# ChrisDud0257/SSL

Measured on AMD Instinct MI355X. Metric: SSG-loss edge-pixels/sec (fwd+bwd) 3x256x256 k_s=25 k_w=9, higher is better.
Workload: dtype f32; 1 GPU; C2: batch 16 x 3x256x256 per GPU, Laplacian mask, k_s=25 k_w=9 sigma=1.0, L1+KL w=1e3, SSGs materialised; launch=per-kernel, ranks_seen=1, edge_px_rank0=76466, images_rank0=16, input_checksum=c1391ff6908574f6, gradient_accumulation=fixed-point integer atomics (bit-reproducible, the shipped default), prewarm_steps=1949, parallelism=images sharded x1, no data-path collective

## Files before the change

include/ssg_hip.h:

```cpp
#ifndef SSG_HIP_H
#define SSG_HIP_H

#include <stddef.h>
#include <stdint.h>

#ifdef __cplusplus
extern "C" {
#endif

typedef void *ssg_stream_t;

#define SSG_E_BADARG (-1)
#define SSG_E_TOOLARGE (-2)
#define SSG_E_WORKSPACE (-3)
#define SSG_E_IMAGESMALL (-4)
#define SSG_E_ALIGN (-5)
#define SSG_E_PLAN (-6)

int ssg_abi_version(void);
const char *ssg_status_string(int status);
int ssg_device_status(ssg_stream_t stream);

int ssg_set_operator_plan_threshold(int positions);
int ssg_operator_pool_trim(void);
int ssg_compute_similarity(const float *image, const int *pos, float *out,
                           int mc, int psize, int ksize, int height, int width,
                           int channel, ssg_stream_t stream);

int ssg_compute_similarity_backward(const float *image, const float *grads,
                                    const int *pos, float *image_grads, int mc,
                                    int psize, int ksize, int height, int width,
                                    int channel, ssg_stream_t stream);

size_t ssg_edge_scratch_bytes(int B, int H, int W);
size_t ssg_forward_plan_bytes(int B, int H, int W, int capacity);
int ssg_set_dense_threshold(int edge_pixels_per_tile);
int ssg_set_overlap(int mode);
int ssg_last_overlap_assignment(void);
int ssg_set_tiny_step(int on);
int ssg_edge_list(const void *mask, int mask_kind, int mask_channels, int B,
                  int H, int W, int mask_stride, float lap_threshold,
                  int plan_ks ,
                  int *edges, int capacity, int *counts,
                  int *rank_map , int *tile_order ,
                  int *fwd_plan , void *scratch,
                  ssg_stream_t stream);

int ssg_edge_mask_laplacian(const float *gt, int B, int H, int W,
                            float lap_threshold, int mask_stride,
                            uint8_t *mask_out, ssg_stream_t stream);

int ssg_map_forward(const float *img, const float *img2, int B, int C, int H,
                    int W, const int *edges, const int *tile_order ,
                    const int *rank_map ,
// ... 113 lines not shown
```

ssl_amd/_lib.py:

```python
import ctypes
import os
import subprocess

_HERE = os.path.dirname(os.path.abspath(__file__))
CSRC = os.path.join(_HERE, "csrc")
SO_PATH = os.path.join(CSRC, "libssg_hip.so")
PROF_SO_PATH = os.path.join(CSRC, "libssg_hip_prof.so")
HEADER = os.path.join(os.path.dirname(_HERE), "include", "ssg_hip.h")

_vp, _i, _f, _sz = ctypes.c_void_p, ctypes.c_int, ctypes.c_float, ctypes.c_size_t

PROTOTYPES = {
    "ssg_abi_version": (_i, []),
    "ssg_status_string": (ctypes.c_char_p, [_i]),
    "ssg_compute_similarity": (_i, [_vp, _vp, _vp, _i, _i, _i, _i, _i, _i, _vp]),
    "ssg_compute_similarity_backward": (_i, [_vp, _vp, _vp, _vp, _i, _i, _i, _i, _i, _i, _vp]),
    "ssg_edge_scratch_bytes": (_sz, [_i, _i, _i]),
    "ssg_forward_plan_bytes": (_sz, [_i, _i, _i, _i]),
    "ssg_set_dense_threshold": (_i, [_i]),
    "ssg_set_overlap": (_i, [_i]),
    "ssg_last_overlap_assignment": (_i, []),
    "ssg_set_tiny_step": (_i, [_i]),
    "ssg_edge_list": (_i, [_vp, _i, _i, _i, _i, _i, _i, _f, _i, _vp, _i, _vp, _vp, _vp, _vp, _vp, _vp]),
    "ssg_edge_mask_laplacian": (_i, [_vp, _i, _i, _i, _f, _i, _vp, _vp]),
    "ssg_map_forward": (_i, [_vp, _vp, _i, _i, _i, _i, _vp, _vp, _vp, _vp, _vp, _i, _i, _i, _f, _f, _i, _vp, _vp,
                             _vp, _vp]),
    "ssg_backward_scratch_bytes": (_sz, [_i, _i]),
    "ssg_map_backward": (_i, [_vp, _i, _i, _i, _i, _vp, _vp, _vp, _vp, _vp, _i, _i, _i, _f, _i, _vp, _vp, _vp, _vp,
                              _vp, _vp]),
    "ssg_grad_fix_bytes": (_sz, [_i, _i, _i, _i]),
    "ssg_loss_scratch_bytes": (_sz, [_i, _i, _i, _i, _i]),
    "ssg_loss_backward": (_i, [_vp, _i, _i, _i, _i, _vp, _vp, _vp, _vp, _vp, _i, _i, _i, _f, _i, _vp, _vp, _f, _f,
                               _vp, _vp, _vp, _vp, _vp, _vp, _i, _vp]),
    "ssg_loss_workspace_bytes": (_sz, [_i, _i, _i, _i, _i]),
    "ssg_loss_rows_bytes": (_sz, [_i, _i]),
    "ssg_loss_tm_bytes": (_sz, [_i, _i]),
    "ssg_loss_workspace_layout": (_i, [_i, _i, _i, _i, _i, _i, ctypes.POINTER(ctypes.c_size_t)]),
# ... 102 lines not shown
```

ssl_amd/csrc/ssg_api.hip:

```cpp
#include "../../include/ssg_hip.h"

#include <atomic>
#include <cstdlib>
#include <mutex>

#include "ssg_common.hpp"

namespace ssg {
int launch_fwd(const FwdParams &p, hipStream_t st);
int launch_bwd(const BwdParams &p, hipStream_t st);
unsigned bwd_grid(const BwdParams &p);
size_t bwd_max_partials(int B, int H, int W, int n_rows);
int launch_loss_finalize(const LossFinalize &f, hipStream_t st);
const char *fwd_kernel_name(int ks, int kw);
const char *bwd_kernel_name(int ks, int kw);
size_t edge_scratch_bytes(int B, int H, int W);
int launch_edge_list(const void *mask, int kind, int mask_channels, int B, int H, int W, int stride, float thr,
                     int *edges, int capacity, int *counts, int *rank, int *order, int *plan, int dense_thr,
                     int plan_tile_rows, void *scratch, void *zero_a, size_t zero_a_bytes, void *zero_b,
                     size_t zero_b_bytes, void *zero_c, size_t zero_c_bytes, hipStream_t st);
size_t fwd_plan_bytes(int B, int H, int W, int capacity);
int fwd_plan_order_offset(int B, int H, int W);
struct DenseParams {
  const float *img[2];
  float *out[2];
  int nimg;
  const int *rank;
  const int *n_dense;
  const int *tiles;
  int max_tiles;
  const int *n_dev;
  int n_host;
  int B, H, W;
  float sigma, eps;
  int generalization;
  int dbg;
  double *row_scale;
  float *tm[2];
  int tm_slots;
  int grid_tiles;
  const int *strips;
  int max_strips;
  int *status;
  int raw;
};
int fwd_plan_strip_offset(int B, int H, int W);
int dense_max_strips(int B, int H, int W, int ks);
bool dense_supported(int ks, int kw, int C);
int dense_max_tiles(int B, int H, int W, int ks);
int dense_tile_rows(int ks);
int launch_fwd_dense(const DenseParams &p, int ks, int kw, int C, hipStream_t st);
int launch_edge_mask(const float *gt, int B, int H, int W, float thr, int stride, uint8_t *out, hipStream_t st);
bool grow_supported(int ks, int kw);
unsigned grow_grid(int n_host);
int launch_grad_rows(const GrowParams &p, int ks, int kw, hipStream_t st);
int launch_rows_tm(const TmRowsParams &p, int ks, int kw, hipStream_t st);
int rows_tm_parts(int n_tiles);
int launch_pos_to_mask(const int *pos, int mc, int Hp, int Wp, uint8_t *mask, hipStream_t st);
int launch_pos_relabel(const int *pos, int mc, int Hp, int Wp, int *rank, int *perm, int *dup, int *ndup, int *plan,
                       int *order2, hipStream_t st);
// ... 27 lines not shown

constexpr int DENSE_THR_DEFAULT = 16;
static std::atomic<int> g_dense_thr{-1};
static int dense_threshold() {
  int v = g_dense_thr.load(std::memory_order_relaxed);
  if (v < 0) {
    v = env_int("SSG_DENSE_THR", DENSE_THR_DEFAULT);
    if (v < 0) v = 0;
    g_dense_thr.store(v, std::memory_order_relaxed);
  }
  return v;
}

static std::atomic<int> g_tiny_step{1};
extern "C" int ssg_set_tiny_step(int on) { return g_tiny_step.exchange(on != 0 ? 1 : 0, std::memory_order_relaxed); }
extern "C" int ssg_set_operator_plan_threshold(int positions);
extern "C" int ssg_set_dense_threshold(int edge_pixels_per_tile) {
  const int prev = dense_threshold();
  g_dense_thr.store(edge_pixels_per_tile > 0 ? edge_pixels_per_tile : 0, std::memory_order_relaxed);
  return prev;
}

#ifdef SSG_PROFILE
static std::atomic<int> g_dbg{-1};
static int dbg_mask() {
  int v = g_dbg.load(std::memory_order_relaxed);
  if (v < 0) {
    v = env_int("SSG_DEBUG_SKIP", 0);
    if (v < 0) v = 0;
    g_dbg.store(v, std::memory_order_relaxed);
// ... 81 lines not shown
int *plan_hint_device_word(hipStream_t st) {
  if (overlap_mode() != 3) return nullptr;
  return plan_hint(stream_capturing(st)).dev;
}
}

struct Schedule {
  hipStream_t st = nullptr;
  bool may_fork = false;
  int assign = 0;
  bool chains = false;
  bool gated = false;
  int rows_hint = 0;
  SideStream *side = nullptr;
  bool open = false;
  hipStream_t dense() const { return open && assign == 2 ? side->side : st; }
  hipStream_t direct() const { return open && assign == 1 ? side->side : st; }
};

static Schedule schedule(hipStream_t st, int ks, bool chains) {
  Schedule s;
  s.st = st;
  const int mode = overlap_mode();
  int n_sparse = -1, n_tiles = -1;
  if (mode == 3) {
    const PlanHint h = plan_hint(true);
    if (h.host) {
      n_sparse = ((volatile int *)h.host)[0];
      n_tiles = ((volatile int *)h.host)[1];
    }
// ... 73 lines not shown

static int bwd_qsplit() {
  static int v = -1;
  if (v < 0) {
    v = env_int("SSG_BWD_QSPLIT", 0);
    if (v < 0) v = 0;
    if (v > 25) v = 25;
  }
  return v;
}

static size_t split_scratch_bytes(int n_rows, int ks) {
  const size_t n = (size_t)(n_rows > 0 ? n_rows : 1);
  return align_up(sizeof(float) * n * ks * ks, 256) + 3 * align_up(sizeof(float) * n, 256);
}

struct TileMajor {
  float *rows[2] = {nullptr, nullptr};
  int slots = 0;
};
static bool strips_enabled() {
  static int v = -1;
  if (v < 0) {
    v = env_int("SSG_STRIPS", 1) != 0;
  }
  return v != 0;
}
static bool tile_major_enabled() {
  static int v = -1;
  if (v < 0) {
// ... 3 lines not shown
}

static int split_tm_tiles(const BwdParams &p, const TileMajor *tm) {
  if (!tm || tm->slots <= 0) return 0;
  const int mt = dense_max_tiles(p.B, p.H, p.W, p.ks);
  return tm->slots < mt ? tm->slots : mt;
}

static bool split_row_classes(const BwdParams &p, int n_tm) {
  return p.mode == GRAD_LOSS && n_tm == 0 && p.row_scale && p.ks <= 25;
}

static int split_backward(BwdParams p, const int *rank, const int *plan, void *scratch, Schedule &sc,
                          const LossFinalize *fin = nullptr, bool *fin_done = nullptr, const TileMajor *tm = nullptr) {
  const hipStream_t st = sc.st;
  float *G = (float *)scratch;
  const size_t nfl = align_up(sizeof(float) * (size_t)(p.n_host > 0 ? p.n_host : 1), 256);
  float *sum_b = (float *)((char *)scratch + align_up(sizeof(float) * (size_t)p.n_host * p.ks * p.ks, 256));
  float *gmax_part = (float *)((char *)sum_b + nfl);
  float *dot = (float *)((char *)gmax_part + nfl);
  const int n_tm = split_tm_tiles(p, tm);
  GrowParams g{};
  g.mode = p.mode;
  g.gin = p.gin;
  g.ssg = p.ssg;
  g.ssg2 = p.ssg2;
  g.row_scale = p.row_scale;
  g.rows_scratch = p.rows_scratch;
  g.n_dev = p.n_dev;
  g.n_host = p.n_host;
  g.C = p.C;
  g.sigma = p.sigma;
  g.generalization = p.generalization;
  g.w_l1 = p.w_l1;
  g.w_kl = p.w_kl;
// ... 10 lines not shown
  }
  const size_t n_fix = (size_t)p.B * p.C * p.H * p.W;
  const bool apriori = p.gfix && p.mode == GRAD_LOSS && n_tm == 0;
  const bool classes = split_row_classes(p, n_tm);
  if (sc.chains && !sc.open && classes && p.grad) fork_side(sc, dbg_mask() & ((1 << 27) | (1 << 28) | (1 << 29)));
  const bool gated = sc.open && sc.gated;
  if (apriori) {
    g.gmax_part = nullptr;
    g.fix_word = (unsigned *)(p.gfix + n_fix);
  }
  int rc = gated ? (int)hipEventRecord(sc.side->gate, st) : 0;
  if (!rc && !(dbg_mask() & (1 << 29))) {
    if (classes) {
      GrowParams gd = g;
      gd.only = 1;
      rc = launch_grad_rows(gd, p.ks, p.kw, sc.dense());
      GrowParams gs = g;
      gs.only = 2;
      gs.grid_cap = 4096;
      gs.tm_hdr = plan + 1;
      gs.tm_slots = 0;
      gs.sparse_order = plan + fwd_plan_order_offset(p.B, p.H, p.W);
      gs.partials = p.partials + 2 * (size_t)grow_grid(p.n_host);
      if (!rc) rc = launch_grad_rows(gs, p.ks, p.kw, sc.direct());
    } else {
      rc = launch_grad_rows(g, p.ks, p.kw, st);
    }
  }
  if (!rc && n_tm > 0) {
    TmRowsParams t{};
    t.tm[0] = tm->rows[0];
// ... 354 lines not shown
}

int ssg_edge_list(const void *mask, int mask_kind, int mask_channels, int B, int H, int W, int mask_stride,
                  float lap_threshold, int plan_ks, int *edges, int capacity, int *counts, int *rank_map,
                  int *tile_order, int *fwd_plan, void *scratch, ssg_stream_t stream) {
  return edge_list_impl(mask, mask_kind, mask_channels, B, H, W, mask_stride, lap_threshold, plan_ks, edges, capacity,
                        counts, rank_map, tile_order, fwd_plan, scratch, nullptr, 0, nullptr, 0, nullptr, 0, stream);
}

int ssg_edge_mask_laplacian(const float *gt, int B, int H, int W, float lap_threshold, int mask_stride,
                            uint8_t *mask_out, ssg_stream_t stream) {
  if (!gt || !mask_out || B <= 0 || H <= 0 || W <= 0) return SSG_E_BADARG;
  return launch_edge_mask(gt, B, H, W, lap_threshold, mask_stride, mask_out, (hipStream_t)stream);
}

static int map_forward_impl(const float *img, const float *img2, int B, int C, int H, int W, const int *edges,
                            const int *tile_order, const int *rank_map, const int *fwd_plan, const int *n_edges_dev,
                            int n_rows, int ks, int kw, float sigma, float eps, int generalization, float *ssg,
                            float *ssg2, double *row_scale, bool row_scale_zeroed, Schedule &sc,
                            const TileMajor *tm = nullptr) {
  if (n_rows < 0 || !sizes_ok(ks, kw) || B <= 0 || C <= 0) return SSG_E_BADARG;
  if (H <= ks / 2 || W <= ks / 2) return SSG_E_IMAGESMALL;
  if (n_rows == 0) return 0;
  if (!img || !edges || !ssg || ((img2 != nullptr) != (ssg2 != nullptr))) return SSG_E_BADARG;
  FwdParams p{};
  p.img[0] = img;
  p.img[1] = img2;
  p.out[0] = ssg;
  p.out[1] = ssg2;
  p.nimg = img2 ? 2 : 1;
  p.edges = edges;
  p.estride = 3;
  p.order = tile_order;
  p.n_dev = n_edges_dev;
  p.n_host = n_rows;
// ... 18 lines not shown
    d.rank = rank_map;
    d.n_dense = fwd_plan + 1;
    d.tiles = fwd_plan + 4;
    d.max_tiles = dense_max_tiles(B, H, W, ks);
    d.n_dev = n_edges_dev;
    d.n_host = n_rows;
    d.B = B;
    d.H = H;
    d.W = W;
    d.sigma = sigma;
    d.eps = eps;
    d.generalization = generalization;
    d.dbg = (dbg_mask() >> 16) & 0xff;
    d.row_scale = row_scale;
    d.status = device_status_word();
    if (tm && tm->slots > 0 && row_scale && img2) {
      d.tm[0] = tm->rows[0];
      d.tm[1] = tm->rows[1];
      d.tm_slots = tm->slots;
      d.max_strips = strips_enabled() ? dense_max_strips(B, H, W, ks) : 0;
      d.strips = d.max_strips ? fwd_plan + fwd_plan_strip_offset(B, H, W) : nullptr;
    }
    if (row_scale && !row_scale_zeroed) {
      const int rc0 = (int)hipMemsetAsync(row_scale, 0, sizeof(double) * 2 * (size_t)n_rows, sc.st);
      if (rc0) return rc0;
    }
    fork_side(sc, dbg_mask() & ((1 << 25) | (1 << 26)));
    int rc = (dbg_mask() & (1 << 25)) ? 0 : launch_fwd_dense(d, ks, kw, C, sc.dense());
    p.order = fwd_plan + fwd_plan_order_offset(B, H, W);
    p.n_dev = fwd_plan;
// ... 51 lines not shown
    Schedule sc = schedule((hipStream_t)stream, ks, false);
    rc = split_backward(p, rank_map, fwd_plan, scratch, sc);
  } else {
    if (p.gfix) rc = launch_grad_fix_bound(p, (hipStream_t)stream);
    if (!rc) rc = launch_bwd(p, (hipStream_t)stream);
  }
  return rc ? rc : det_end(p, (hipStream_t)stream);
}

size_t ssg_grad_fix_bytes(int B, int C, int H, int W) { return sizeof(long long) * ((size_t)B * C * H * W + 8); }

static size_t partials_bytes(int B, int H, int W, int n_rows) {
  return align_up(2 * sizeof(float) * bwd_max_partials(B, H, W, n_rows) + 64, 256);
}

size_t ssg_loss_scratch_bytes(int B, int H, int W, int n_rows, int ks) {
  return partials_bytes(B, H, W, n_rows) + split_scratch_bytes(n_rows, ks);
}

static int loss_backward(const float *sr, int B, int C, int H, int W, const int *edges, const int *tile_order,
                         const int *rank_map, const int *fwd_plan, const int *n_edges_dev, int n_rows, int ks, int kw,
                         float sigma, int generalization, float *ssg_sr, float *ssg_gt, float w_l1, float w_kl,
                         const float *upstream, float *loss_out, float *grad_sr, void *scratch, void *grad_fix,
                         const double *row_scale, bool rows_scratch, bool fix_zeroed, bool grad_is_output,
                         Schedule &sc, const TileMajor *tm = nullptr, bool nan_on_overflow = false) {
  if (n_rows < 0 || !sizes_ok(ks, kw) || B <= 0 || C <= 0 || !loss_out) return SSG_E_BADARG;
  if (H <= ks / 2 || W <= ks / 2) return SSG_E_IMAGESMALL;
  const hipStream_t st = sc.st;
  if (n_rows == 0) return (int)hipMemsetAsync(loss_out, 0, 2 * sizeof(float), st);
  if (!sr || !edges || !ssg_sr || !ssg_gt || !scratch) return SSG_E_BADARG;
  BwdParams p{};
  p.img = sr;
// ... 17 lines not shown
  p.partials = (float *)scratch;
  p.upstream = upstream;
  p.ks = ks;
  p.kw = kw;
  p.dbg = (dbg_mask() >> 8) & 0xff;
  p.row_scale = row_scale;
  p.rows_scratch = rows_scratch ? 1 : 0;
  const bool split = split_ok(ks, kw, C, rank_map, fwd_plan, scratch);
  if (row_scale && !split) return SSG_E_BADARG;
  int rc = det_begin(p, grad_fix, st, fix_zeroed);
  if (rc) return rc;
  const int n_tm = split ? split_tm_tiles(p, tm) : 0;
  const int nparts = !split ? (int)bwd_grid(p)
                            : (split_row_classes(p, n_tm) ? 2 : 1) * (int)grow_grid(n_rows) + rows_tm_parts(n_tm);
  const int set_size = split && n_tm == 0 ? (int)grow_grid(n_rows) : 0;
  const LossFinalize fin{p.partials, nparts, n_edges_dev, n_rows, ks * ks, w_l1, w_kl, loss_out, nan_on_overflow ? 1 : 0, set_size};
  bool fin_done = false;
  if (split) {
    rc = split_backward(p, rank_map, fwd_plan, (char *)scratch + partials_bytes(B, H, W, n_rows), sc, &fin, &fin_done, tm);
  } else {
    p.fix_inline = p.gfix ? 1 : 0;
    rc = launch_bwd(p, st);
  }
  const int fin_reads = set_size > 0 ? (nparts / set_size) * ((n_rows + 3) / 4) : nparts;
  if (!rc) rc = det_end(p, st, grad_is_output, (fin_done || fin_reads > 8192) ? nullptr : &fin, &fin_done);
  if (rc || fin_done) return rc;
  return launch_loss_finalize(fin, st);
}

int ssg_loss_backward(const float *sr, int B, int C, int H, int W, const int *edges, const int *tile_order,
                      const int *rank_map, const int *fwd_plan, const int *n_edges_dev, int n_rows, int ks, int kw,
                      float sigma, int generalization,
                      float *ssg_sr, float *ssg_gt, float w_l1, float w_kl, const float *upstream,
                      float *loss_out, float *grad_sr, void *scratch, void *grad_fix, const double *row_scale,
                      int rows_are_scratch, ssg_stream_t stream) {
  Schedule sc = schedule((hipStream_t)stream, ks, true);
  const int rc = loss_backward(sr, B, C, H, W, edges, tile_order, rank_map, fwd_plan, n_edges_dev, n_rows, ks, kw, sigma,
                               generalization, ssg_sr, ssg_gt, w_l1, w_kl, upstream, loss_out, grad_sr, scratch,
                               grad_fix, row_scale, rows_are_scratch != 0, false, false, sc);
// ... 132 lines not shown
    t.dbg = env_int("SSG_TINY_DBG", 0);
    return launch_tiny_step(t, C, (hipStream_t)stream);
  }
  int *order = (int *)(ws + lw.order);
  int *plan = (int *)(ws + lw.plan);
  void *escratch = ws + lw.escratch;
  void *lscratch = ws + lw.lscratch;
  double *row_scale = (double *)(ws + lw.row_scale);
  const bool defer = split_ok(ks, kw, C, rank, plan, lscratch) && dense_supported(ks, kw, C);
  if (!defer) tm.slots = 0;
  if (defer) order = nullptr;
  if (!dense_supported(ks, kw, C)) plan = nullptr;
  const bool zero_fix = grad_fix && grad_sr;
  Schedule sc = schedule((hipStream_t)stream, ks, defer && grad_sr);
  const size_t fix_bytes = sizeof(long long) * ((size_t)B * C * H * W + 8), rs_bytes = 2 * sizeof(double) * (size_t)capacity;
  int rc = edge_list_impl(mask_kind == 2 ? (const void *)gt : mask, mask_kind, mask_kind == 2 ? 3 : mask_channels, B, H,
                          W, mask_stride, lap_threshold, ks, edges, capacity, counts, rank, order, plan, escratch,
                          defer ? (void *)row_scale : nullptr, rs_bytes, zero_fix ? grad_fix : nullptr, fix_bytes,
                          (grad_is_output && grad_sr && !zero_fix) ? (void *)grad_sr : nullptr,
                          sizeof(float) * (size_t)B * C * H * W, stream);
  if (!rc && grad_is_output && grad_sr && !zero_fix && ((sizeof(float) * (size_t)B * C * H * W) & 15))
    rc = (int)hipMemsetAsync((char *)grad_sr + ((sizeof(float) * (size_t)B * C * H * W) & ~(size_t)15), 0,
                             (sizeof(float) * (size_t)B * C * H * W) & 15, (hipStream_t)stream);
  if (rc) return rc;
  rc = map_forward_impl(sr, gt, B, C, H, W, edges, order, rank, plan, counts, capacity, ks, kw, sigma, eps,
                        generalization, ssg_sr, ssg_gt, defer ? row_scale : nullptr, defer, sc, &tm);
  if (!rc)
    rc = loss_backward(sr, B, C, H, W, edges, order, rank, plan, counts, capacity, ks, kw, sigma, generalization,
                       ssg_sr, ssg_gt, w_l1, w_kl, nullptr, loss_out, grad_sr, lscratch, grad_fix,
                       defer ? row_scale : nullptr, fused, zero_fix, grad_is_output && zero_fix, sc, &tm, true);
  const int rcj = join_side(sc);
  return rc ? rc : rcj;
}

int ssg_loss_fwd_bwd(const float *sr, const float *gt, const void *mask, int mask_kind, int mask_channels, int B,
                     int C, int H, int W, int ks, int kw, float sigma, float eps, int generalization, float w_l1,
                     float w_kl, int mask_stride, float lap_threshold, int capacity, float *ssg_sr, float *ssg_gt,
                     int *counts, float *loss_out, float *grad_sr, void *workspace, size_t workspace_bytes,
                     void *grad_fix, ssg_stream_t stream) {
  return loss_fwd_bwd_impl(sr, gt, mask, mask_kind, mask_channels, B, C, H, W, ks, kw, sigma, eps, generalization, w_l1,
                           w_kl, mask_stride, lap_threshold, capacity, ssg_sr, ssg_gt, counts, loss_out, grad_sr,
// ... 103 lines not shown
```

ssl_amd/csrc/ssg_bwd.hip:

```cpp
#include "ssg_common.hpp"

namespace ssg {

template <int BS, int KW>
__device__ __forceinline__ void shared_window_sums(const float (&v)[BS + KW - 1], float (&out)[BS]) {
  static_assert(BS <= KW, "windows must overlap in at least one tap");
  float mid = v[BS - 1];
#pragma unroll
  for (int k = BS; k < KW; ++k) mid += v[k];
  float suf[BS], pre[BS];
  suf[BS - 1] = 0.f;
#pragma unroll
  for (int j = BS - 2; j >= 0; --j) suf[j] = (j == BS - 2) ? v[j] : v[j] + suf[j + 1];
  pre[0] = 0.f;
#pragma unroll
  for (int j = 1; j < BS; ++j) pre[j] = (j == 1) ? v[KW] : pre[j - 1] + v[KW - 1 + j];
#pragma unroll
  for (int j = 0; j < BS; ++j) {
    float t = mid;
    if (j < BS - 1) t += suf[j];
    if (j > 0) t += pre[j];
    out[j] = t;
  }
}
// ... 588 lines not shown
    double a = 0, b = 0;
    for (int sset = 0; sset < nsets; ++sset) {
      const float2 *pp = (const float2 *)f.partials + (size_t)sset * set_size;
      int i = vt;
      for (; i + 3 * 1024 < live; i += 4 * 1024) {
        const float2 v0 = pp[i], v1 = pp[i + 1024], v2 = pp[i + 2048], v3 = pp[i + 3072];
        a += (double)v0.x + (double)v1.x + (double)v2.x + (double)v3.x;
        b += (double)v0.y + (double)v1.y + (double)v2.y + (double)v3.y;
      }
      for (; i < live; i += 1024) {
        const float2 v = pp[i];
        a += (double)v.x;
        b += (double)v.y;
      }
    }
    s1[vt] = a;
    s2[vt] = b;
  }
  __syncthreads();
  for (int o = 512; o > 0; o >>= 1) {
    for (int vt = threadIdx.x; vt < o; vt += NT) {
      s1[vt] += s1[vt + o];
      s2[vt] += s2[vt + o];
    }
    __syncthreads();
  }
  if (threadIdx.x == 0) {
    const int nrows = rows_to_do(f.n_dev, f.n_host);
    const double M = (double)nrows * (double)f.P;
    f.loss_out[0] = nrows > 0 ? (float)((double)f.w_l1 * s1[0] / M) : 0.f;
// ... 191 lines not shown
```

ssl_amd/csrc/ssg_common.hpp:

```cpp
#pragma once
#include <hip/hip_runtime.h>
#include <hip/amd_detail/amd_hip_unsafe_atomics.h>
#include <stdint.h>

#include <atomic>
#include <type_traits>
#include <utility>

#ifdef SSG_PROFILE
#define SSG_DBG(p, bits) ((p).dbg & (bits))
#else
#define SSG_DBG(p, bits) 0
#endif

namespace ssg {

__device__ __forceinline__ int reflect_idx(int i, int n) {
  i = i < 0 ? -i : i;
  return i >= n ? 2 * n - 2 - i : i;
}

__device__ __forceinline__ int reflect101_idx(int i, int n) {
  if (n == 1) return 0;
  i = i < 0 ? -i : i;
// ... 156 lines not shown
    kl = qnan;
    g = qnan;
  }
  return g;
}

struct LossFinalize {
  const float *partials;
  int nparts;
  const int *n_dev;
  int n_host, P;
  float w_l1, w_kl;
  float *loss_out;
  int nan_on_overflow;
  int set_size;
};

inline int env_int(const char *name, int dflt) {
#ifdef SSG_PROFILE
  const char *e = getenv(name);
  return e ? atoi(e) : dflt;
#else
  (void)name;
  return dflt;
#endif
}

template <class K>
inline int ensure_dynamic_lds(K kernel, int bytes, std::atomic<unsigned long long> &done) {
  int dev = 0;
// ... 160 lines not shown
  float *loss_out;
  int *ticket;
  int nan_on_overflow;
  int dbg;
};

__device__ __forceinline__ int rows_to_do(const int *n_dev, int n_host) {
  int n = n_host;
  if (n_dev) {
    const int d = *n_dev;
    n = d < n ? d : n;
  }
  return n;
}

}

#ifdef SSG_PROFILE
namespace ssg { void prof_poison_lds(hipStream_t st); }
#undef hipLaunchKernelGGL
#define hipLaunchKernelGGL(kernelName, numBlocks, numThreads, memPerBlock, streamId, ...)                         \
  do {                                                                                                            \
    ::ssg::prof_poison_lds(streamId);                                                                             \
    kernelName<<<(numBlocks), (numThreads), (memPerBlock), (streamId)>>>(__VA_ARGS__);                            \
  } while (0)
#endif
```

ssl_amd/csrc/ssg_dense.hip:

```cpp
#include "ssg_common.hpp"

namespace ssg {

typedef float f2 __attribute__((ext_vector_type(2)));

template <int D>
__device__ __forceinline__ float quad_next(float v) {
  constexpr int ctrl = D == 1 ? 0xF9 : 0xFE;
  return __builtin_bit_cast(float, __builtin_amdgcn_update_dpp(0, __builtin_bit_cast(int, v), ctrl, 0xf, 0xf, true));
}

template <int LO, int LEN, typename T, int N>
__device__ __forceinline__ T block_sum(const T (&e)[N]) {
  static_assert(LEN >= 1 && (LEN & (LEN - 1)) == 0 && LO >= 0 && LO + LEN <= N, "power-of-two block inside the array");
  if constexpr (LEN == 1) return e[LO];
  else return block_sum<LO, LEN / 2>(e) + block_sum<LO + LEN / 2, LEN / 2>(e);
}
constexpr int floor_pow2(int n) { return n < 2 ? 1 : 2 * floor_pow2(n / 2); }
template <int LO, int LEN, typename T, int N>
__device__ __forceinline__ T sum_from(const T (&e)[N]) {
  constexpr int B = floor_pow2(LEN);
  if constexpr (B == LEN) return block_sum<LO, LEN>(e);
  else return block_sum<LO, B>(e) + sum_from<LO + B, LEN - B>(e);
}
// ... 7 lines not shown
template <int KW>
__device__ __forceinline__ float tap_sum(const float (&v)[KW], const float (&w)[KW], float rest) {
  static_assert(KW % 2 == 1 && KW >= 5, "pairs of taps and a last one");
  constexpr int NP = KW / 2;
  f2 a = f2{v[0], v[1]} * f2{w[0], w[1]}, b = f2{v[2], v[3]} * f2{w[2], w[3]};
#pragma unroll
  for (int j = 2; j < NP; ++j) {
    const f2 vv = f2{v[2 * j], v[2 * j + 1]}, ww = f2{w[2 * j], w[2 * j + 1]};
    if (j % 2 == 0) a = __builtin_elementwise_fma(vv, ww, a);
    else b = __builtin_elementwise_fma(vv, ww, b);
  }
  const f2 r2 = a + b;
  return (r2.x + r2.y) + __builtin_fmaf(w[KW - 1], v[KW - 1], rest);
}

struct DenseParams {
  const float *img[2];
  float *out[2];
  int nimg;
  const int *rank;
  const int *n_dense;
  const int *tiles;
  int max_tiles;
  const int *n_dev;
  int n_host;
  int B, H, W;
  float sigma, eps;
  int generalization;
  int dbg;
  double *row_scale;
  float *tm[2];
  int tm_slots;
  int grid_tiles;
  const int *strips;
  int max_strips;
  int *status;
  int raw;
};

constexpr int DT_X = 32;
constexpr int dense_lane_px(int kw) { return kw == 9 ? 10 : 12; }
constexpr bool dense_h_paired(int kw) { return kw == 9; }
constexpr int dense_h_group(int kw) { return kw == 9 ? 10 : 12; }
constexpr int dense_h_stride(int kw) { return kw == 9 ? 40 : 49; }
__device__ __forceinline__ int dense_h_col(int ex, int L, int G, bool paired) {
  const int k = ex % L;
  return paired ? G * (ex / L) + 2 * (k % (L / 2)) + k / (L / 2) : ex;
}

template <int KS, int KW, int C, int NW, bool TM = false, bool RAW = false, int NCH = 0>
__device__ __forceinline__ void fwd_dense_body(const DenseParams &p) {
  static_assert(!(TM && RAW), "raw distances go to the caller's row-major rows");
  constexpr int NT = 64 * NW;
  constexpr int HP = KS / 2, HK = KW / 2, P = KS * KS, HALO = HP + HK, DT_Y = 16 - 2 * HK;
  constexpr int RH = DT_Y + 2 * HALO, RWD = DT_X + 2 * HALO, RS = RWD + 1;
  constexpr int UH = DT_Y + 2 * HK, UW = DT_X + 2 * HK;
  constexpr int L = dense_lane_px(KW), HL = L / 2;
  constexpr int NV = HL + KW - 1;
  constexpr int DT_HS = dense_h_stride(KW);
  constexpr bool HPAIR = dense_h_paired(KW);
  constexpr int HG = dense_h_group(KW);
  constexpr int NE_MAX = DT_Y * DT_X, NCHUNK = NCH > 0 ? NCH : NE_MAX / 64;
// ... 3 lines not shown
  static_assert(UH == 16 && DT_X == 32 && 4 * L >= UW && 3 * HG + L <= DT_HS && HG >= L && (HPAIR || HG == L) && L % 2 == 0 && KW - 1 <= L,
                "lane map: 16 U-rows x 4 column groups (one quad) of L pixels; a window spans two lanes");

  extern __shared__ __attribute__((aligned(16))) float smem[];
  float *reg = smem;
  float *F = reg + C * RH * RS;
  float *HF = F + UH * UW;
  float *Hb = HF + UH * DT_HS;
  double *rsum = (double *)Hb;
  constexpr int RSTR = UH * DT_HS / 2;
  static_assert(NE_MAX <= RSTR, "row sums alias the wave's H buffer");
  int *elist = (int *)(Hb + NW * UH * DT_HS);
  int *misc = elist + NE_MAX * 3;

  const int tid = threadIdx.x, lane = tid & 63, wv = tid >> 6;
  const int tslot = blockIdx.x / p.nimg, which = blockIdx.x - tslot * p.nimg;
  if (tslot >= dense_tile_count(p.n_dense)) return;
  if (p.tm_slots > 0 && tm_active(p.n_dense, p.tm_slots, rows_to_do(p.n_dev, p.n_host)) != TM) return;
  if (TM && p.tm_slots <= 0) return;
  if (p.n_dense[1] != DT_Y) {
    if (p.status && tid == 0) atomicOr(p.status, 1);
    return;
  }
  const int H = p.H, W = p.W;
  const int tx_n = (W + DT_X - 1) / DT_X, ty_n = (H + DT_Y - 1) / DT_Y;
  const int listed = dense_tile_at(p.n_dense, p.tiles, p.B * ty_n * tx_n, tslot);
  if (TM && p.strips && (listed & TILE_IN_STRIP)) return;
  if constexpr (NCH > 0) {
    if (((listed & TILE_HUGE) != 0) != (NCH > 2)) return;
  }
// ... 442 lines not shown
#pragma unroll
  for (int ck = 0; ck < NCHUNK; ++ck)
    if (ck * 64 + lane < n_e) rsum[wv * RSTR + ck * 64 + lane] = rs[ck];
  __threadfence_block();
  __syncthreads();
  if (RAW || !p.generalization || SSG_DBG(p, 8)) return;
  if (p.row_scale) {
    double *rsc = p.row_scale + (size_t)which * p.n_host;
    for (int e = tid; e < n_e; e += NT) {
      if (elist[3 * e + 2] < 0) continue;
      double tot = 0.0;
#pragma unroll
      for (int k = 0; k < NW; ++k) tot += rsum[k * RSTR + e];
      const double sc = 1.0 / (tot + (double)p.eps);
      rsc[elist[3 * e + 2]] = TM ? -sc : sc;
    }
    return;
  }
  if constexpr (TM) return;
  asm volatile("s_waitcnt vmcnt(0)" ::: "memory");
  __syncthreads();
  constexpr int RPL = (P + 63) / 64;
  for (int e0 = 2 * wv; e0 < n_e; e0 += 2 * NW) {
    float v[2][RPL];
    double scale[2];
    float *o[2];
    bool ok[2];
#pragma unroll
    for (int j = 0; j < 2; ++j) {
      const int e = e0 + j < n_e ? e0 + j : e0;
// ... 522 lines not shown
```

ssl_amd/csrc/ssg_grow.hip:

```cpp
#include "ssg_common.hpp"

namespace ssg {

template <int KS, int KW>
__global__ __launch_bounds__(256) void ssg_grad_rows(GrowParams p) {
  constexpr int P = KS * KS, HP = KS / 2, HK = KW / 2, EPL = (P + 63) / 64;
  __shared__ float sred[12];
  const int lane = threadIdx.x & 63, wv = threadIdx.x >> 6;
  const int nrows = rows_to_do(p.n_dev, p.n_host);
  if (p.fix_word && blockIdx.x == 0 && threadIdx.x == 0) {
    *p.fix_word = __float_as_uint(loss_grad_bound(p.sigma, p.C, KW, p.w_l1, p.w_kl, p.upstream, nrows, P));
  }
  const bool via_list = p.tm_hdr && p.sparse_order && (p.only == 2 || tm_active(p.tm_hdr, p.tm_slots, nrows));
  const int n_list = via_list ? (p.tm_hdr[-1] < nrows ? p.tm_hdr[-1] : nrows) : 0;
  const int live_rows = (nrows + 3) / 4 < p.ngroups ? (nrows + 3) / 4 : p.ngroups;
  const int live_groups = via_list ? (n_list + 3) / 4 : live_rows;
  for (int g = live_groups + blockIdx.x * 256 + threadIdx.x; g < p.ngroups; g += gridDim.x * 256) {
    if (p.gmax_part) p.gmax_part[g] = 0.f;
    if (p.mode == GRAD_LOSS) {
      p.partials[2 * g] = 0.f;
      p.partials[2 * g + 1] = 0.f;
    }
  }
  for (int grp = blockIdx.x; grp < live_groups; grp += gridDim.x) {
  const int k4 = grp * 4 + wv;
  const int n = via_list ? (k4 < n_list ? (p.sparse_order[k4] & ORDER_MASK) : nrows) : k4;
  float l1p = 0.f, klp = 0.f, gmax = 0.f;
  const bool tm_row = n < nrows && p.row_scale && p.mode == GRAD_LOSS && p.row_scale[n] < 0.0;
  const bool other_chain = p.only == 1 && n < nrows && p.row_scale[n] == 0.0;
  if (n < nrows && !tm_row && !other_chain) {
    const size_t base = (size_t)n * P;
    float va[EPL], vg[EPL];
    const float *src_a = p.mode == GRAD_D ? p.gin : p.ssg;
#pragma unroll
    for (int k = 0; k < EPL; ++k) {
      const int e = lane + 64 * k;
      va[k] = e < P ? src_a[base + e] : 0.f;
    }
    if (p.mode != GRAD_D) {
      const float *src_b = p.mode == GRAD_S ? p.gin : p.ssg2;
#pragma unroll
      for (int k = 0; k < EPL; ++k) {
        const int e = lane + 64 * k;
        vg[k] = e < P ? src_b[base + e] : 0.f;
      }
      if (p.row_scale && p.mode == GRAD_LOSS) {
        const double sa = p.row_scale[n], sb2 = p.row_scale[(size_t)p.n_host + n];
        if (sa != 0.0) {
#pragma unroll
          for (int k = 0; k < EPL; ++k) {
            const int e = lane + 64 * k;
            va[k] = (float)(sa * (double)va[k]);
            if (e < P && !p.rows_scratch) const_cast<float *>(p.ssg)[base + e] = va[k];
          }
        }
        if (sb2 != 0.0) {
#pragma unroll
          for (int k = 0; k < EPL; ++k) {
            const int e = lane + 64 * k;
            vg[k] = (float)(sb2 * (double)vg[k]);
            if (e < P && !p.rows_scratch) const_cast<float *>(p.ssg2)[base + e] = vg[k];
          }
        }
      }
      const float invM = 1.f / ((float)nrows * (float)P);
      const float u1 = p.upstream ? p.upstream[0] : 1.f, u2 = p.upstream ? p.upstream[1] : 1.f;
      const float w1m = p.w_l1 * invM * u1, w2m = p.w_kl * invM * u2;
      float dot = 0.f;
#pragma unroll
      for (int k = 0; k < EPL; ++k) {
        const int e = lane + 64 * k;
        float g = 0.f;
        if (e < P) g = p.mode == GRAD_S ? vg[k] : criteria_elem(va[k], vg[k], w1m, w2m, l1p, klp);
        vg[k] = g;
        dot = __builtin_fmaf(g, va[k], dot);
      }
      dot = p.generalization ? wave_sum(dot) : 0.f;
      const float kfac = 1.f / (p.sigma * (float)(p.C * KW * KW));
#pragma unroll
      for (int k = 0; k < EPL; ++k) va[k] = -(va[k] * kfac) * (vg[k] - dot);
    }
    float sb = 0.f, gm = 0.f;
#pragma unroll
    for (int k = 0; k < EPL; ++k) {
      const int e = lane + 64 * k;
      if (e < P) {
        const int py = e / KS, px = e - py * KS;
        if (e == HP * KS + HP) va[k] = 0.f;
        gm = fmaxf(gm, fabsf(va[k]));
        const bool border = py < HK || py > KS - 1 - HK || px < HK || px > KS - 1 - HK;
        if (border) sb += va[k];
// ... 523 lines not shown
```

ssl_amd/engine.py:

```python
import torch

from . import _lib


def _ptr(t):
    return None if t is None else t.data_ptr()


def _stream():
    return torch.cuda.current_stream().cuda_stream


def _need_gpu(*tensors):
    for t in tensors:
        if t is not None and not t.is_cuda:
            raise RuntimeError(f"ssl_amd: expected a GPU tensor, got device {t.device}; the SSG engine has no CPU path")


def _f32c(t):
    return t.detach().to(torch.float32).contiguous()


def deterministic_default():
    import os
# ... 70 lines not shown
    return EdgeList(edges, counts, rank, order, plan, ks)


def set_overlap(mode):
    return _lib.lib().ssg_set_overlap(int(mode))


def set_dense_threshold(edge_pixels_per_tile):
    return _lib.lib().ssg_set_dense_threshold(int(edge_pixels_per_tile))


def set_tiny_step(on):
    return bool(_lib.lib().ssg_set_tiny_step(int(bool(on))))


def edge_mask_laplacian(gt, lap_threshold=20.0, mask_stride=0):
    _need_gpu(gt)
    g = _f32c(gt)
    B, C, H, W = g.shape
    if C != 3:
        raise ValueError("Laplacian edge mask needs a 3-channel image")
    out = torch.empty((B, H, W), dtype=torch.uint8, device=g.device)
    with torch.cuda.device(g.device):
        _lib.check(_lib.lib().ssg_edge_mask_laplacian(_ptr(g), B, H, W, float(lap_threshold), int(mask_stride or 0),
                                                      _ptr(out), _stream()))
    return out


class _SSGMapFn(torch.autograd.Function):

# ... 359 lines not shown
```

Measured before the change: 65.90 million edge-px/s.

## Fold dense-tile loss-gradient row pass into the dense forward kernel epilogue

Adds a per-tile ticket so the last image block finishing a dense tile runs the loss-gradient row computation (criteria, dot, G and border sums) directly in the forward kernel epilogue. This skips the separate dense-class grad_rows launch and writes per-tile L1/KL partials that the loss finalize kernel also reduces. The row-gradient logic is factored into a shared templated helper. The fold is on by default for ks=25, kw=9, C=3. It costs extra scratch, an atomic ticket per tile, and serialised tail work on one block per tile, which could lengthen the forward kernel.

```diff
diff --git a/include/ssg_hip.h b/include/ssg_hip.h
--- a/include/ssg_hip.h
+++ b/include/ssg_hip.h
@@ -38,6 +38,7 @@
 int ssg_set_overlap(int mode);
 int ssg_last_overlap_assignment(void);
 int ssg_set_tiny_step(int on);
+int ssg_set_dense_row_fold(int on);
 int ssg_edge_list(const void *mask, int mask_kind, int mask_channels, int B,
                   int H, int W, int mask_stride, float lap_threshold,
                   int plan_ks ,
diff --git a/ssl_amd/_lib.py b/ssl_amd/_lib.py
--- a/ssl_amd/_lib.py
+++ b/ssl_amd/_lib.py
@@ -21,6 +21,7 @@
     "ssg_set_overlap": (_i, [_i]),
     "ssg_last_overlap_assignment": (_i, []),
     "ssg_set_tiny_step": (_i, [_i]),
+    "ssg_set_dense_row_fold": (_i, [_i]),
     "ssg_edge_list": (_i, [_vp, _i, _i, _i, _i, _i, _i, _f, _i, _vp, _i, _vp, _vp, _vp, _vp, _vp, _vp]),
     "ssg_edge_mask_laplacian": (_i, [_vp, _i, _i, _i, _f, _i, _vp, _vp]),
     "ssg_map_forward": (_i, [_vp, _vp, _i, _i, _i, _i, _vp, _vp, _vp, _vp, _vp, _i, _i, _i, _f, _f, _i, _vp, _vp,
diff --git a/ssl_amd/csrc/ssg_api.hip b/ssl_amd/csrc/ssg_api.hip
--- a/ssl_amd/csrc/ssg_api.hip
+++ b/ssl_amd/csrc/ssg_api.hip
@@ -21,29 +21,6 @@
                      size_t zero_b_bytes, void *zero_c, size_t zero_c_bytes, hipStream_t st);
 size_t fwd_plan_bytes(int B, int H, int W, int capacity);
 int fwd_plan_order_offset(int B, int H, int W);
-struct DenseParams {
-  const float *img[2];
-  float *out[2];
-  int nimg;
-  const int *rank;
-  const int *n_dense;
-  const int *tiles;
-  int max_tiles;
-  const int *n_dev;
-  int n_host;
-  int B, H, W;
-  float sigma, eps;
-  int generalization;
-  int dbg;
-  double *row_scale;
-  float *tm[2];
-  int tm_slots;
-  int grid_tiles;
-  const int *strips;
-  int max_strips;
-  int *status;
-  int raw;
-};
 int fwd_plan_strip_offset(int B, int H, int W);
 int dense_max_strips(int B, int H, int W, int ks);
 bool dense_supported(int ks, int kw, int C);
@@ -101,6 +78,10 @@
 
 static std::atomic<int> g_tiny_step{1};
 extern "C" int ssg_set_tiny_step(int on) { return g_tiny_step.exchange(on != 0 ? 1 : 0, std::memory_order_relaxed); }
+static std::atomic<int> g_dense_row_fold{1};
+extern "C" int ssg_set_dense_row_fold(int on) {
+  return g_dense_row_fold.exchange(on != 0 ? 1 : 0, std::memory_order_relaxed);
+}
 extern "C" int ssg_set_operator_plan_threshold(int positions);
 extern "C" int ssg_set_dense_threshold(int edge_pixels_per_tile) {
   const int prev = dense_threshold();
@@ -212,6 +193,7 @@
   int rows_hint = 0;
   SideStream *side = nullptr;
   bool open = false;
+  bool fold = false;
   hipStream_t dense() const { return open && assign == 2 ? side->side : st; }
   hipStream_t direct() const { return open && assign == 1 ? side->side : st; }
 };
@@ -315,6 +297,18 @@
   const size_t n = (size_t)(n_rows > 0 ? n_rows : 1);
   return align_up(sizeof(float) * n * ks * ks, 256) + 3 * align_up(sizeof(float) * n, 256);
 }
+struct SplitScratch {
+  float *G, *sum_b, *gmax_part, *dot;
+};
+static SplitScratch carve_split(void *scratch, int n_host, int ks) {
+  SplitScratch s;
+  const size_t nfl = align_up(sizeof(float) * (size_t)(n_host > 0 ? n_host : 1), 256);
+  s.G = (float *)scratch;
+  s.sum_b = (float *)((char *)scratch + align_up(sizeof(float) * (size_t)n_host * ks * ks, 256));
+  s.gmax_part = (float *)((char *)s.sum_b + nfl);
+  s.dot = (float *)((char *)s.gmax_part + nfl);
+  return s;
+}
 
 struct TileMajor {
   float *rows[2] = {nullptr, nullptr};
@@ -348,11 +342,8 @@
 static int split_backward(BwdParams p, const int *rank, const int *plan, void *scratch, Schedule &sc,
                           const LossFinalize *fin = nullptr, bool *fin_done = nullptr, const TileMajor *tm = nullptr) {
   const hipStream_t st = sc.st;
-  float *G = (float *)scratch;
-  const size_t nfl = align_up(sizeof(float) * (size_t)(p.n_host > 0 ? p.n_host : 1), 256);
-  float *sum_b = (float *)((char *)scratch + align_up(sizeof(float) * (size_t)p.n_host * p.ks * p.ks, 256));
-  float *gmax_part = (float *)((char *)sum_b + nfl);
-  float *dot = (float *)((char *)gmax_part + nfl);
+  const SplitScratch ss = carve_split(scratch, p.n_host, p.ks);
+  float *G = ss.G, *sum_b = ss.sum_b, *gmax_part = ss.gmax_part, *dot = ss.dot;
   const int n_tm = split_tm_tiles(p, tm);
   GrowParams g{};
   g.mode = p.mode;
@@ -393,7 +384,7 @@
     if (classes) {
       GrowParams gd = g;
       gd.only = 1;
-      rc = launch_grad_rows(gd, p.ks, p.kw, sc.dense());
+      if (!sc.fold) rc = launch_grad_rows(gd, p.ks, p.kw, sc.dense());
       GrowParams gs = g;
       gs.only = 2;
       gs.grid_cap = 4096;
@@ -778,11 +769,17 @@
   return launch_edge_mask(gt, B, H, W, lap_threshold, mask_stride, mask_out, (hipStream_t)stream);
 }
 
+struct DenseFold {
+  int *ticket = nullptr;
+  float *partials = nullptr;
+  GrowParams grow{};
+};
+
 static int map_forward_impl(const float *img, const float *img2, int B, int C, int H, int W, const int *edges,
                             const int *tile_order, const int *rank_map, const int *fwd_plan, const int *n_edges_dev,
                             int n_rows, int ks, int kw, float sigma, float eps, int generalization, float *ssg,
                             float *ssg2, double *row_scale, bool row_scale_zeroed, Schedule &sc,
-                            const TileMajor *tm = nullptr) {
+                            const TileMajor *tm = nullptr, const DenseFold *fold = nullptr) {
   if (n_rows < 0 || !sizes_ok(ks, kw) || B <= 0 || C <= 0) return SSG_E_BADARG;
   if (H <= ks / 2 || W <= ks / 2) return SSG_E_IMAGESMALL;
   if (n_rows == 0) return 0;
@@ -831,6 +828,11 @@
     d.dbg = (dbg_mask() >> 16) & 0xff;
     d.row_scale = row_scale;
     d.status = device_status_word();
+    if (sc.fold && fold && row_scale && img2) {
+      d.fold_ticket = fold->ticket;
+      d.fold_partials = fold->partials;
+      d.grow = fold->grow;
+    }
     if (tm && tm->slots > 0 && row_scale && img2) {
       d.tm[0] = tm->rows[0];
       d.tm[1] = tm->rows[1];
@@ -912,8 +914,15 @@
   return align_up(2 * sizeof(float) * bwd_max_partials(B, H, W, n_rows) + 64, 256);
 }
 
+static size_t fold_ticket_bytes(int B, int H, int W, int ks) {
+  return ks == 25 ? align_up(sizeof(int) * (size_t)dense_max_tiles(B, H, W, ks), 256) : 0;
+}
+static size_t fold_bytes(int B, int H, int W, int ks) {
+  return ks == 25 ? align_up(2 * sizeof(float) * (size_t)dense_max_tiles(B, H, W, ks), 256) + fold_ticket_bytes(B, H, W, ks) : 0;
+}
+
 size_t ssg_loss_scratch_bytes(int B, int H, int W, int n_rows, int ks) {
-  return partials_bytes(B, H, W, n_rows) + split_scratch_bytes(n_rows, ks);
+  return partials_bytes(B, H, W, n_rows) + split_scratch_bytes(n_rows, ks) + fold_bytes(B, H, W, ks);
 }
 
 static int loss_backward(const float *sr, int B, int C, int H, int W, const int *edges, const int *tile_order,
@@ -961,7 +970,14 @@
   const int nparts = !split ? (int)bwd_grid(p)
                             : (split_row_classes(p, n_tm) ? 2 : 1) * (int)grow_grid(n_rows) + rows_tm_parts(n_tm);
   const int set_size = split && n_tm == 0 ? (int)grow_grid(n_rows) : 0;
-  const LossFinalize fin{p.partials, nparts, n_edges_dev, n_rows, ks * ks, w_l1, w_kl, loss_out, nan_on_overflow ? 1 : 0, set_size};
+  LossFinalize fin{p.partials, nparts, n_edges_dev, n_rows, ks * ks, w_l1, w_kl, loss_out, nan_on_overflow ? 1 : 0, set_size};
+  if (sc.fold) {
+    fin.partials = p.partials + 2 * (size_t)grow_grid(n_rows);
+    fin.nparts = (int)grow_grid(n_rows);
+    fin.tile_partials = (const float *)((char *)scratch + partials_bytes(B, H, W, n_rows) + split_scratch_bytes(n_rows, ks));
+    fin.tile_hdr = fwd_plan + 1;
+    fin.max_tiles = dense_max_tiles(B, H, W, ks);
+  }
   bool fin_done = false;
   if (split) {
     rc = split_backward(p, rank_map, fwd_plan, (char *)scratch + partials_bytes(B, H, W, n_rows), sc, &fin, &fin_done, tm);
@@ -969,7 +985,7 @@
     p.fix_inline = p.gfix ? 1 : 0;
     rc = launch_bwd(p, st);
   }
-  const int fin_reads = set_size > 0 ? (nparts / set_size) * ((n_rows + 3) / 4) : nparts;
+  const int fin_reads = (set_size > 0 ? (fin.nparts / set_size) * ((n_rows + 3) / 4) : nparts) + (sc.fold ? fin.max_tiles : 0);
   if (!rc) rc = det_end(p, st, grad_is_output, (fin_done || fin_reads > 8192) ? nullptr : &fin, &fin_done);
   if (rc || fin_done) return rc;
   return launch_loss_finalize(fin, st);
@@ -1132,9 +1148,35 @@
   const bool zero_fix = grad_fix && grad_sr;
   Schedule sc = schedule((hipStream_t)stream, ks, defer && grad_sr);
   const size_t fix_bytes = sizeof(long long) * ((size_t)B * C * H * W + 8), rs_bytes = 2 * sizeof(double) * (size_t)capacity;
+  sc.fold = defer && ks == 25 && kw == 9 && C == 3 && generalization && g_dense_row_fold.load(std::memory_order_relaxed);
+  DenseFold fold;
+  const size_t ticket_bytes = sc.fold ? fold_ticket_bytes(B, H, W, ks) : 0;
+  if (sc.fold) {
+    const size_t pb = partials_bytes(B, H, W, capacity);
+    const SplitScratch ss = carve_split((char *)lscratch + pb, capacity, ks);
+    fold.ticket = (int *)((char *)row_scale - ticket_bytes);
+    fold.partials = (float *)((char *)lscratch + pb + split_scratch_bytes(capacity, ks));
+    GrowParams &g = fold.grow;
+    g.mode = GRAD_LOSS;
+    g.ssg = ssg_sr;
+    g.ssg2 = ssg_gt;
+    g.row_scale = row_scale;
+    g.rows_scratch = fused ? 1 : 0;
+    g.n_dev = counts;
+    g.n_host = capacity;
+    g.C = C;
+    g.sigma = sigma;
+    g.generalization = generalization;
+    g.w_l1 = w_l1;
+    g.w_kl = w_kl;
+    g.G = grad_sr ? ss.G : nullptr;
+    g.sum_b = grad_sr ? ss.sum_b : nullptr;
+    g.fix_word = zero_fix ? (unsigned *)((long long *)grad_fix + (size_t)B * C * H * W) : nullptr;
+  }
   int rc = edge_list_impl(mask_kind == 2 ? (const void *)gt : mask, mask_kind, mask_kind == 2 ? 3 : mask_channels, B, H,
                           W, mask_stride, lap_threshold, ks, edges, capacity, counts, rank, order, plan, escratch,
-                          defer ? (void *)row_scale : nullptr, rs_bytes, zero_fix ? grad_fix : nullptr, fix_bytes,
+                          defer ? (void *)((char *)row_scale - ticket_bytes) : nullptr, ticket_bytes + rs_bytes,
+                          zero_fix ? grad_fix : nullptr, fix_bytes,
                           (grad_is_output && grad_sr && !zero_fix) ? (void *)grad_sr : nullptr,
                           sizeof(float) * (size_t)B * C * H * W, stream);
   if (!rc && grad_is_output && grad_sr && !zero_fix && ((sizeof(float) * (size_t)B * C * H * W) & 15))
@@ -1142,7 +1184,7 @@
                              (sizeof(float) * (size_t)B * C * H * W) & 15, (hipStream_t)stream);
   if (rc) return rc;
   rc = map_forward_impl(sr, gt, B, C, H, W, edges, order, rank, plan, counts, capacity, ks, kw, sigma, eps,
-                        generalization, ssg_sr, ssg_gt, defer ? row_scale : nullptr, defer, sc, &tm);
+                        generalization, ssg_sr, ssg_gt, defer ? row_scale : nullptr, defer, sc, &tm, &fold);
   if (!rc)
     rc = loss_backward(sr, B, C, H, W, edges, order, rank, plan, counts, capacity, ks, kw, sigma, generalization,
                        ssg_sr, ssg_gt, w_l1, w_kl, nullptr, loss_out, grad_sr, lscratch, grad_fix,
diff --git a/ssl_amd/csrc/ssg_bwd.hip b/ssl_amd/csrc/ssg_bwd.hip
--- a/ssl_amd/csrc/ssg_bwd.hip
+++ b/ssl_amd/csrc/ssg_bwd.hip
@@ -626,6 +626,14 @@
         b += (double)v.y;
       }
     }
+    if (f.tile_partials) {
+      const int nt = dense_tile_count(f.tile_hdr) < f.max_tiles ? dense_tile_count(f.tile_hdr) : f.max_tiles;
+      for (int i = vt; i < nt; i += 1024) {
+        const float2 v = ((const float2 *)f.tile_partials)[i];
+        a += (double)v.x;
+        b += (double)v.y;
+      }
+    }
     s1[vt] = a;
     s2[vt] = b;
   }
diff --git a/ssl_amd/csrc/ssg_common.hpp b/ssl_amd/csrc/ssg_common.hpp
--- a/ssl_amd/csrc/ssg_common.hpp
+++ b/ssl_amd/csrc/ssg_common.hpp
@@ -194,6 +194,9 @@
   float *loss_out;
   int nan_on_overflow;
   int set_size;
+  const float *tile_partials;
+  const int *tile_hdr;
+  int max_tiles;
 };
 
 inline int env_int(const char *name, int dflt) {
@@ -384,6 +387,113 @@
   return n;
 }
 
+struct DenseParams {
+  const float *img[2];
+  float *out[2];
+  int nimg;
+  const int *rank;
+  const int *n_dense;
+  const int *tiles;
+  int max_tiles;
+  const int *n_dev;
+  int n_host;
+  int B, H, W;
+  float sigma, eps;
+  int generalization;
+  int dbg;
+  double *row_scale;
+  float *tm[2];
+  int tm_slots;
+  int grid_tiles;
+  const int *strips;
+  int max_strips;
+  int *status;
+  int raw;
+  int *fold_ticket;
+  float *fold_partials;
+  GrowParams grow;
+};
+
+template <int KS, int KW, int R>
+__device__ __forceinline__ void grad_loss_rows(const GrowParams &p, const int (&n)[R], int nrows, int lane, float &l1p,
+                                               float &klp, float &gmax) {
+#pragma clang fp contract(off)
+  constexpr int P = KS * KS, HP = KS / 2, HK = KW / 2, EPL = (P + 63) / 64;
+  float va[R][EPL], vg[R][EPL];
+#pragma unroll
+  for (int j = 0; j < R; ++j) {
+    const size_t base = (size_t)(n[j] >= 0 ? n[j] : 0) * P;
+#pragma unroll
+    for (int k = 0; k < EPL; ++k) {
+      const int e = lane + 64 * k;
+      va[j][k] = n[j] >= 0 && e < P ? p.ssg[base + e] : 0.f;
+    }
+#pragma unroll
+    for (int k = 0; k < EPL; ++k) {
+      const int e = lane + 64 * k;
+      vg[j][k] = n[j] >= 0 && e < P ? p.ssg2[base + e] : 0.f;
+    }
+  }
+  const float invM = 1.f / ((float)nrows * (float)P);
+  const float u1 = p.upstream ? p.upstream[0] : 1.f, u2 = p.upstream ? p.upstream[1] : 1.f;
+  const float w1m = p.w_l1 * invM * u1, w2m = p.w_kl * invM * u2;
+  const float kfac = 1.f / (p.sigma * (float)(p.C * KW * KW));
+#pragma unroll
+  for (int j = 0; j < R; ++j) {
+    if (n[j] < 0) continue;
+    const size_t base = (size_t)n[j] * P;
+    if (p.row_scale) {
+      const double sa = p.row_scale[n[j]], sb2 = p.row_scale[(size_t)p.n_host + n[j]];
+      if (sa != 0.0) {
+#pragma unroll
+        for (int k = 0; k < EPL; ++k) {
+          const int e = lane + 64 * k;
+          va[j][k] = (float)(sa * (double)va[j][k]);
+          if (e < P && !p.rows_scratch) const_cast<float *>(p.ssg)[base + e] = va[j][k];
+        }
+      }
+      if (sb2 != 0.0) {
+#pragma unroll
+        for (int k = 0; k < EPL; ++k) {
+          const int e = lane + 64 * k;
+          vg[j][k] = (float)(sb2 * (double)vg[j][k]);
+          if (e < P && !p.rows_scratch) const_cast<float *>(p.ssg2)[base + e] = vg[j][k];
+        }
+      }
+    }
+    float dot = 0.f;
+#pragma unroll
+    for (int k = 0; k < EPL; ++k) {
+      const int e = lane + 64 * k;
+      float g = 0.f;
+      if (e < P) g = criteria_elem(va[j][k], vg[j][k], w1m, w2m, l1p, klp);
+      vg[j][k] = g;
+      dot = __builtin_fmaf(g, va[j][k], dot);
+    }
+    dot = p.generalization ? wave_sum(dot) : 0.f;
+#pragma unroll
+    for (int k = 0; k < EPL; ++k) va[j][k] = -(va[j][k] * kfac) * (vg[j][k] - dot);
+    float sb = 0.f, gm = 0.f;
+#pragma unroll
+    for (int k = 0; k < EPL; ++k) {
+      const int e = lane + 64 * k;
+      if (e < P) {
+        const int py = e / KS, px = e - py * KS;
+        if (e == HP * KS + HP) va[j][k] = 0.f;
+        gm = fmaxf(gm, fabsf(va[j][k]));
+        const bool border = py < HK || py > KS - 1 - HK || px < HK || px > KS - 1 - HK;
+        if (border) sb += va[j][k];
+        if (p.G) p.G[base + e] = va[j][k];
+      }
+    }
+    if (p.sum_b) {
+      sb = wave_sum(sb);
+      if (lane == 0) p.sum_b[n[j]] = sb;
+    }
+    gmax = fmaxf(gmax, gm);
+  }
+}
+
 }
 
 #ifdef SSG_PROFILE
diff --git a/ssl_amd/csrc/ssg_dense.hip b/ssl_amd/csrc/ssg_dense.hip
--- a/ssl_amd/csrc/ssg_dense.hip
+++ b/ssl_amd/csrc/ssg_dense.hip
@@ -45,29 +45,7 @@
   return (r2.x + r2.y) + __builtin_fmaf(w[KW - 1], v[KW - 1], rest);
 }
 
-struct DenseParams {
-  const float *img[2];
-  float *out[2];
-  int nimg;
-  const int *rank;
-  const int *n_dense;
-  const int *tiles;
-  int max_tiles;
-  const int *n_dev;
-  int n_host;
-  int B, H, W;
-  float sigma, eps;
-  int generalization;
-  int dbg;
-  double *row_scale;
-  float *tm[2];
-  int tm_slots;
-  int grid_tiles;
-  const int *strips;
-  int max_strips;
-  int *status;
-  int raw;
-};
+
 
 constexpr int DT_X = 32;
 constexpr int dense_lane_px(int kw) { return kw == 9 ? 10 : 12; }
@@ -77,6 +55,41 @@
 __device__ __forceinline__ int dense_h_col(int ex, int L, int G, bool paired) {
   const int k = ex % L;
   return paired ? G * (ex / L) + 2 * (k % (L / 2)) + k / (L / 2) : ex;
+}
+
+template <int KS, int KW, int NW, int R>
+__device__ __forceinline__ void fold_rows_epilogue(const DenseParams &p, const int *elist, int *misc, int n_e, int tslot,
+                                                   int nrows) {
+  static_assert(NW == 4, "the criteria sums of four waves: misc[8..15]");
+  const int tid = threadIdx.x, lane = tid & 63, wv = tid >> 6;
+  asm volatile("s_waitcnt vmcnt(0)" ::: "memory");
+  __syncthreads();
+  if (tid == 0) misc[NW + 1] = __hip_atomic_fetch_add(p.fold_ticket + tslot, 1, __ATOMIC_ACQ_REL, __HIP_MEMORY_SCOPE_AGENT);
+  __syncthreads();
+  if (misc[NW + 1] != p.nimg - 1) return;
+  __threadfence();
+  float l1p = 0.f, klp = 0.f, gmax = 0.f;
+  for (int e0 = R * wv; e0 < n_e; e0 += R * NW) {
+    int rows[R];
+#pragma unroll
+    for (int j = 0; j < R; ++j) {
+      const int r = e0 + j < n_e ? elist[3 * (e0 + j) + 2] : -1;
+      rows[j] = r < nrows ? r : -1;
+    }
+    grad_loss_rows<KS, KW, R>(p.grow, rows, nrows, lane, l1p, klp, gmax);
+  }
+  l1p = wave_sum(l1p);
+  klp = wave_sum(klp);
+  float *sred = (float *)(misc + 8);
+  if (lane == 0) {
+    sred[wv] = l1p;
+    sred[4 + wv] = klp;
+  }
+  __syncthreads();
+  if (tid == 0) {
+    p.fold_partials[2 * tslot] = (sred[0] + sred[1]) + (sred[2] + sred[3]);
+    p.fold_partials[2 * tslot + 1] = (sred[4] + sred[5]) + (sred[6] + sred[7]);
+  }
 }
 
 template <int KS, int KW, int C, int NW, bool TM = false, bool RAW = false, int NCH = 0>
@@ -110,6 +123,11 @@
   int *misc = elist + NE_MAX * 3;
 
   const int tid = threadIdx.x, lane = tid & 63, wv = tid >> 6;
+  if constexpr (!TM && !RAW && NCH > 0) {
+    if (p.fold_ticket && p.grow.fix_word && blockIdx.x == 0 && tid == 0)
+      *p.grow.fix_word = __float_as_uint(loss_grad_bound(p.grow.sigma, p.grow.C, KW, p.grow.w_l1, p.grow.w_kl,
+                                                         p.grow.upstream, rows_to_do(p.n_dev, p.n_host), KS * KS));
+  }
   const int tslot = blockIdx.x / p.nimg, which = blockIdx.x - tslot * p.nimg;
   if (tslot >= dense_tile_count(p.n_dense)) return;
   if (p.tm_slots > 0 && tm_active(p.n_dense, p.tm_slots, rows_to_do(p.n_dev, p.n_host)) != TM) return;
@@ -582,6 +600,9 @@
       for (int k = 0; k < NW; ++k) tot += rsum[k * RSTR + e];
       const double sc = 1.0 / (tot + (double)p.eps);
       rsc[elist[3 * e + 2]] = TM ? -sc : sc;
+    }
+    if constexpr (!TM && !RAW && NCH > 0) {
+      if (p.fold_ticket) fold_rows_epilogue<KS, KW, NW, (NCHUNK > 2 ? 1 : 2)>(p, elist, misc, n_e, tslot, nrows);
     }
     return;
   }
diff --git a/ssl_amd/csrc/ssg_grow.hip b/ssl_amd/csrc/ssg_grow.hip
--- a/ssl_amd/csrc/ssg_grow.hip
+++ b/ssl_amd/csrc/ssg_grow.hip
@@ -28,7 +28,10 @@
   float l1p = 0.f, klp = 0.f, gmax = 0.f;
   const bool tm_row = n < nrows && p.row_scale && p.mode == GRAD_LOSS && p.row_scale[n] < 0.0;
   const bool other_chain = p.only == 1 && n < nrows && p.row_scale[n] == 0.0;
-  if (n < nrows && !tm_row && !other_chain) {
+  if (n < nrows && !tm_row && !other_chain && p.mode == GRAD_LOSS) {
+    const int rows[1] = {n};
+    grad_loss_rows<KS, KW, 1>(p, rows, nrows, lane, l1p, klp, gmax);
+  } else if (n < nrows && !tm_row && !other_chain) {
     const size_t base = (size_t)n * P;
     float va[EPL], vg[EPL];
     const float *src_a = p.mode == GRAD_D ? p.gin : p.ssg;
@@ -37,44 +40,15 @@
       const int e = lane + 64 * k;
       va[k] = e < P ? src_a[base + e] : 0.f;
     }
-    if (p.mode != GRAD_D) {
-      const float *src_b = p.mode == GRAD_S ? p.gin : p.ssg2;
+    if (p.mode == GRAD_S) {
 #pragma unroll
       for (int k = 0; k < EPL; ++k) {
         const int e = lane + 64 * k;
-        vg[k] = e < P ? src_b[base + e] : 0.f;
-      }
-      if (p.row_scale && p.mode == GRAD_LOSS) {
-        const double sa = p.row_scale[n], sb2 = p.row_scale[(size_t)p.n_host + n];
-        if (sa != 0.0) {
-#pragma unroll
-          for (int k = 0; k < EPL; ++k) {
-            const int e = lane + 64 * k;
-            va[k] = (float)(sa * (double)va[k]);
-            if (e < P && !p.rows_scratch) const_cast<float *>(p.ssg)[base + e] = va[k];
-          }
-        }
-        if (sb2 != 0.0) {
-#pragma unroll
-          for (int k = 0; k < EPL; ++k) {
-            const int e = lane + 64 * k;
-            vg[k] = (float)(sb2 * (double)vg[k]);
-            if (e < P && !p.rows_scratch) const_cast<float *>(p.ssg2)[base + e] = vg[k];
-          }
-        }
-      }
-      const float invM = 1.f / ((float)nrows * (float)P);
-      const float u1 = p.upstream ? p.upstream[0] : 1.f, u2 = p.upstream ? p.upstream[1] : 1.f;
-      const float w1m = p.w_l1 * invM * u1, w2m = p.w_kl * invM * u2;
+        vg[k] = e < P ? p.gin[base + e] : 0.f;
+      }
       float dot = 0.f;
 #pragma unroll
-      for (int k = 0; k < EPL; ++k) {
-        const int e = lane + 64 * k;
-        float g = 0.f;
-        if (e < P) g = p.mode == GRAD_S ? vg[k] : criteria_elem(va[k], vg[k], w1m, w2m, l1p, klp);
-        vg[k] = g;
-        dot = __builtin_fmaf(g, va[k], dot);
-      }
+      for (int k = 0; k < EPL; ++k) dot = __builtin_fmaf(vg[k], va[k], dot);
       dot = p.generalization ? wave_sum(dot) : 0.f;
       const float kfac = 1.f / (p.sigma * (float)(p.C * KW * KW));
 #pragma unroll
diff --git a/ssl_amd/engine.py b/ssl_amd/engine.py
--- a/ssl_amd/engine.py
+++ b/ssl_amd/engine.py
@@ -108,6 +108,10 @@
     return bool(_lib.lib().ssg_set_tiny_step(int(bool(on))))
 
 
+def set_dense_row_fold(on):
+    return bool(_lib.lib().ssg_set_dense_row_fold(int(bool(on))))
+
+
 def edge_mask_laplacian(gt, lap_threshold=20.0, mask_stride=0):
     _need_gpu(gt)
     g = _f32c(gt)
```

Measured after the change: 37.16 million edge-px/s, median of 2. 0.564x the previous value.
